# Purpurax/mcaat

Hardware: AMD Instinct MI355X
Metric: k-mers/sec through sdbg_build+cycle_finder, 1B-node graph @ 1/2/4/8 GPUs (higher is better)
Workload: dtype u64

## Files before the change

mcaat_amd/csrc/node_counter.hip:

```cpp
#include <hipcub/hipcub.hpp>

#include <algorithm>
#include <cstdio>
#include <cstdlib>
#include <ctime>
#include <functional>
#include <memory>
#include <mutex>
#include <type_traits>

#include "desc_canon.h"
#include "internal.h"

namespace mcaat {

namespace {

constexpr int kBlock = 256;


struct SkParams {
    int E;
    int m;
    int w;
    int nmax;
    int l2_bits;
    uint64_t salt;
    uint32_t mini;
};

__device__ __forceinline__ uint64_t desc_window(uint64_t w0, uint64_t w1, int i, int E) {
    uint64_t v;
    if (i == 0) v = w0;
    else if (i < 32) v = (w0 >> (2 * i)) | (w1 << (64 - 2 * i));
    else v = w1 >> (2 * (i - 32));
    return v & mask_bits(2 * E);
}

__device__ __forceinline__ uint32_t rev2_32(uint32_t x) {
    x = ((x >> 2) & 0x33333333u) | ((x & 0x33333333u) << 2);
    x = ((x >> 4) & 0x0F0F0F0Fu) | ((x & 0x0F0F0F0Fu) << 4);
    return __builtin_bswap32(x);
}
__device__ __forceinline__ uint32_t mix32(uint32_t x) {
    x ^= x >> 16;
    x *= 0x7feb352du;
    x ^= x >> 15;
    x *= 0x846ca68bu;
    x ^= x >> 16;
    return x;
}

__device__ __forceinline__ uint32_t part_mix(uint32_t h) { return mix32(h ^ 0x70617274u); }

__device__ __forceinline__ uint64_t canon_edge(uint64_t lsb, int E) {
    const uint64_t y = __builtin_bitreverse64(lsb);
    const uint64_t r2 = ((y >> 1) & 0x5555555555555555ULL) | ((y & 0x5555555555555555ULL) << 1);
    const uint64_t rc = (r2 >> (64 - 2 * E)) ^ mask_bits(2 * E);
    return lsb < rc ? lsb : rc;
}

#ifndef MCAAT_AWAVES
#define MCAAT_AWAVES 4
#define MCAAT_ASEG 900
#define MCAAT_APERCU 3
#endif
#ifndef MCAAT_HASH
#define MCAAT_HASH 2
#endif
constexpr int kAWaves = MCAAT_AWAVES;
constexpr int kAThreads = kAWaves * 64;
constexpr int kAPerCu = MCAAT_APERCU;
constexpr int kItem = 127;
constexpr int kCk = 8;
constexpr int kSeg = MCAAT_ASEG;
constexpr int kStage = kSeg * kAWaves;
static_assert(kAThreads >= 256, "threads < 256 own one L1 bucket each");
static_assert(kSeg > 64 * kCk, "a segment must hold a worst-case step");
static_assert(kStage <= 65536, "perm holds 16-bit stage indices");

struct ItemSrc {
    const uint64_t *offsets;
    uint64_t n_reads;
    uint64_t fixed_len;
    uint64_t ipr;
    const uint64_t *item_base;
    const uint32_t *item_np;
    uint64_t n_items;
};

__device__ __forceinline__ void get_item(const ItemSrc &s, int E, uint64_t it, uint64_t &base, int &np) {
    if (s.fixed_len) {
        const uint64_t r = it / s.ipr, c = it - r * s.ipr;
        const uint64_t npos = s.fixed_len - E + 1;
        base = r * s.fixed_len + c * kItem;
        const uint64_t rem = npos - c * kItem;
        np = (int)(rem < (uint64_t)kItem ? rem : kItem);
    } else {
        base = s.item_base[it];
        np = (int)s.item_np[it];
    }
}

struct __attribute__((aligned(8))) u64x2 {
    uint64_t a, b;
};

__device__ __forceinline__ uint64_t rev2_dev(uint64_t x) {
    const uint32_t lo = __builtin_bitreverse32((uint32_t)(x >> 32)), hi = __builtin_bitreverse32((uint32_t)x);
    const uint32_t l = ((lo >> 1) & 0x55555555u) | ((lo << 1) & 0xAAAAAAAAu);
    const uint32_t h = ((hi >> 1) & 0x55555555u) | ((hi << 1) & 0xAAAAAAAAu);
    return ((uint64_t)h << 32) | l;
}

__device__ __forceinline__ uint64_t win32(uint64_t a, uint64_t b, uint64_t B) {
    const int sh = 2 * (int)(B & 31);
    return sh ? (a >> sh) | (b << (64 - sh)) : a;
}

#ifndef MCAAT_HTOP
#define MCAAT_HTOP 1
#endif
template <bool FULL>
__device__ __forceinline__ void hash_step(uint64_t win, int m, uint32_t mmask, uint32_t salt, uint32_t *h) {
#if MCAAT_HTOP
    const int lo = 32 - 2 * m;
    const uint64_t Wt = win << lo;
    const uint64_t R = rev2_dev(win) ^ ~0ULL;
    const uint32_t wl = (uint32_t)Wt, wh = (uint32_t)(Wt >> 32);
    const uint32_t rl = (uint32_t)R, rh = (uint32_t)(R >> 32);
    (void)mmask;
#pragma unroll
    for (int t = 0; t < kCk; ++t) {
        const uint32_t f = t ? __builtin_amdgcn_alignbit(wh, wl, 2 * t) : wl;
        const uint32_t r = t ? __builtin_amdgcn_alignbit(rh, rl, 32 - 2 * t) : rh;
        const uint32_t c = FULL ? min(f, r) : min(f, r) >> lo;
#if MCAAT_HASH == 2
        h[t] = (c ^ salt) * 0x9E3779B1u;
#elif MCAAT_HASH == 1
        uint32_t x = (c ^ salt) * 0x9E3779B1u;
        h[t] = x ^ (x >> 15);
#else
        h[t] = mix32(c ^ salt);
#endif
    }
#else
    const uint64_t R = (rev2_dev(win) ^ ~0ULL) >> (2 * (25 - m));
    const uint32_t wl = (uint32_t)win, wh = (uint32_t)(win >> 32);
    const uint32_t rl = (uint32_t)R, rh = (uint32_t)(R >> 32);
#pragma unroll
    for (int t = 0; t < kCk; ++t) {
        uint32_t f = __builtin_amdgcn_alignbit(wh, wl, 2 * t);
        uint32_t r = __builtin_amdgcn_alignbit(rh, rl, 2 * (kCk - 1 - t));
        if (!FULL) {
            f &= mmask;
            r &= mmask;
        }
#if MCAAT_HASH == 2
        h[t] = (min(f, r) ^ salt) * 0x9E3779B1u;
#elif MCAAT_HASH == 1
        uint32_t x = (min(f, r) ^ salt) * 0x9E3779B1u;
        h[t] = x ^ (x >> 15);
#else
        h[t] = mix32(min(f, r) ^ salt);
#endif
    }
#endif
}

template <int W, int G>
__device__ __forceinline__ void window_min(const uint32_t *H, uint32_t *hm) {
    auto at = [&](int u) { return H[(G * kCk + u) % (3 * kCk)]; };
    if constexpr (W > kCk) {
        uint32_t S[kCk], Pm[W - 1];
        S[kCk - 1] = at(kCk - 1);
#pragma unroll
        for (int t = kCk - 2; t >= 0; --t) S[t] = min(at(t), S[t + 1]);
        Pm[0] = at(kCk);
#pragma unroll
        for (int u = 1; u < W - 1; ++u) Pm[u] = min(Pm[u - 1], at(kCk + u));
#pragma unroll
        for (int t = 0; t < kCk; ++t) hm[t] = min(S[t], Pm[t + W - 1 - kCk]);
    } else {
#pragma unroll
        for (int t = 0; t < kCk; ++t) {
            uint32_t v = at(t);
#pragma unroll
            for (int q = 1; q < W; ++q) v = min(v, at(t + q));
            hm[t] = v;
        }
    }
}

constexpr uint32_t kMiniOne = 1024, kMiniShard = 256;
constexpr uint16_t kDeadSub = 0xffff;


#ifndef MCAAT_WB
#define MCAAT_WB 4
#endif
#ifndef MCAAT_APF
#define MCAAT_APF 1
#endif
constexpr int kAPF = MCAAT_APF;
constexpr int kWB = MCAAT_WB;
#ifndef MCAAT_WPIPE
#define MCAAT_WPIPE 0
#endif
#ifndef MCAAT_CLOSEMASK
#define MCAAT_CLOSEMASK 1
#endif
constexpr bool kWPipe = MCAAT_WPIPE != 0;

constexpr int kPeP = 7, kPePar = 14, kPeLane = 15;

template <int W, bool FULL>
__global__ void __launch_bounds__(kAThreads) k_sk_scatter(const uint64_t *__restrict__ packed, ItemSrc src,
                                                          SkParams P, uint4 *__restrict__ l1_data,
                                                          const uint64_t *__restrict__ l1_base,
                                                          const uint64_t *__restrict__ l1_cap,
                                                          unsigned long long *l1_cursor, uint16_t *__restrict__ l1_sub,
                                                          unsigned long long *prof, unsigned long long *rstate, int rmode) {
    __shared__ uint64_t stage[kStage];
    __shared__ uint8_t stage_l1[kStage];
    __shared__ uint16_t perm[kStage];
    __shared__ uint64_t sbase[kAWaves][2][64];
    __shared__ uint32_t hist[256];
    __shared__ uint32_t boff[256];
    __shared__ uint32_t bcur[256];
    __shared__ unsigned long long rpos[256];
    __shared__ unsigned long long rlim[256];
    __shared__ uint32_t rleft[256];
    __shared__ uint32_t wtot[kAWaves];
    __shared__ int more_flag[2];

    const int wave = threadIdx.x >> 6, lane = threadIdx.x & 63;
    const int tb = threadIdx.x;
    unsigned long long my_next = 0, my_base = 0;
    uint32_t prev_need = 0;
    unsigned long long *rs = rstate ? rstate + ((uint64_t)blockIdx.x * 256 + (tb & 255)) * 3 : nullptr;
    if (tb < 256) {
        hist[tb] = 0;
        bcur[tb] = 0;
        my_base = l1_base[tb];
        rlim[tb] = my_base + l1_cap[tb];
        if (rmode >= 2) {
            rpos[tb] = rs[0];
            rleft[tb] = (uint32_t)rs[1];
            my_next = rs[2];
        } else {
            rleft[tb] = 0;
            my_next = atomicAdd(&l1_cursor[tb], (unsigned long long)P.mini);
        }
    }
    if (threadIdx.x == 0) more_flag[0] = more_flag[1] = 0;
    __syncthreads();
    uint64_t *seg = stage + __builtin_amdgcn_readfirstlane(wave * kSeg);
    uint8_t *seg_l1 = stage_l1 + wave * kSeg;
    uint32_t nflush = 0;

    const int sub_shift = kHShift + kHBits - P.l2_bits;
    auto put = [&](int b, uint64_t pos, const uint4 &d) {
        if (pos < rlim[b]) {
            l1_data[pos] = d;
            const uint64_t hi = (uint64_t)d.w << 32;
            l1_sub[pos] = ((d.w >> (kNShift - 32)) & 63) ? (uint16_t)(sub_shift < 64 ? hi >> sub_shift : 0) : kDeadSub;
        }
    };

    const uint64_t n_items = src.fixed_len ? src.n_reads * src.ipr : src.n_items;
    const uint64_t n_batches = (n_items + 63) / 64;
    const uint64_t bstride = (uint64_t)gridDim.x * kAWaves;
    uint64_t batch = (uint64_t)blockIdx.x * kAWaves + wave;
    constexpr bool kFull = FULL;
    const uint32_t mmask = (uint32_t)mask_bits(2 * P.m);
    const uint32_t salt32 = (uint32_t)P.salt;
    const int nmax = P.nmax;

    uint32_t H[3 * kCk];
    uint64_t cw[3], pa = 0, pb = 0;
    uint64_t qa = 0, qb = 0;
    uint64_t s = 0;
    int np = 0, c = 0, ph = 0, nck = 0;
    uint32_t prev_hm = 0, h_open = 0, p7 = 0, ihc = 0, fill = 0, par = 1, bsf = 0;
    bool active = false;
    auto fetch = [&](uint64_t bt, uint64_t &sb, int &n, uint64_t *w) {
        const uint64_t item = bt * 64 + lane;
        sb = 0;
        n = 0;
        if (bt < n_batches && item < n_items) get_item(src, P.E, item, sb, n);
#pragma unroll
        for (int k = 0; k < 3; ++k) w[k] = packed[(sb >> 5) + k];
    };

    auto step = [&](auto Gc) {
        constexpr int G = decltype(Gc)::value;
        c = __builtin_amdgcn_readfirstlane(c);
        const int rb = kCk * c + 2 * kCk;
        const uint64_t win = win32(pa, pb, s + rb);
        if constexpr (kAPF == 2) {
            pa = qa;
            pb = qb;
            const u64x2 nx = *(const u64x2 *)(packed + ((s + rb + 2 * kCk) >> 5));
            qa = nx.a;
            qb = nx.b;
        } else {
            const u64x2 nx = *(const u64x2 *)(packed + ((s + rb + kCk) >> 5));
            pa = nx.a;
            pb = nx.b;
        }
        hash_step<kFull>(win, P.m, mmask, salt32, H + ((G + 2) % 3) * kCk);
        uint32_t hm[kCk];
        window_min<W, G>(H, hm);
        if (c == 0) {
            prev_hm = hm[0];
            h_open = hm[0];
            p7 = 0;
        }
#if MCAAT_CLOSEMASK
        fill = __builtin_amdgcn_readfirstlane(fill);
#pragma unroll
        for (int t = 0; t < kCk; ++t) {
            const int i = kCk * c + t;
            const uint32_t prv = t ? hm[t - 1] : prev_hm;
            const unsigned long long bm = __builtin_amdgcn_ballot_w64((uint32_t)(i - 1) < (uint32_t)np) &
                                          (__builtin_amdgcn_ballot_w64(i == np) |
                                           __builtin_amdgcn_ballot_w64(hm[t] != prv) |
                                           __builtin_amdgcn_ballot_w64((int)p7 <= (i - nmax) * 128));
            if (bm) {
                if (__builtin_amdgcn_inverse_ballot_w64(bm)) {
                    const uint32_t idx =
                        __builtin_amdgcn_mbcnt_hi((uint32_t)(bm >> 32), __builtin_amdgcn_mbcnt_lo((uint32_t)bm, 0u));
                    seg[fill + idx] = ((uint64_t)(p7 + ihc + (uint32_t)i) << 32) | prv;
                    p7 = (uint32_t)i << kPeP;
                }
                fill += (uint32_t)__popcll(bm);
            }
        }
        (void)h_open;
#else
#pragma unroll
        for (int t = 0; t < kCk; ++t) {
            const int i = kCk * c + t;
            const uint32_t prv = t ? hm[t - 1] : prev_hm;
            const bool cl = ((uint32_t)(i - 1) < (uint32_t)np) &
                            ((i == np) | (hm[t] != prv) | ((int)p7 <= (i - nmax) * 128));
            const unsigned long long bm = __builtin_amdgcn_ballot_w64(cl);
            if (bm) {
                if (cl) {
                    const uint32_t idx =
                        __builtin_amdgcn_mbcnt_hi((uint32_t)(bm >> 32), __builtin_amdgcn_mbcnt_lo((uint32_t)bm, fill));
                    seg[idx] = ((uint64_t)(p7 + ihc + (uint32_t)i) << 32) | h_open;
                    p7 = (uint32_t)i << kPeP;
                    h_open = hm[t];
                }
                fill += (uint32_t)__popcll(bm);
            }
        }
#endif
        prev_hm = hm[kCk - 1];
    };

    unsigned long long tp[5] = {0, 0, 0, 0, 0}, t0 = prof ? __builtin_amdgcn_s_memrealtime() : 0;
    auto tick = [&](int phase) {
        if (prof) {
            const unsigned long long t1 = __builtin_amdgcn_s_memrealtime();
            tp[phase] += t1 - t0;
            t0 = t1;
        }
    };

    auto start_item = [&](auto Gc) {
        constexpr int G = decltype(Gc)::value;
        fetch(batch, s, np, cw);
        par ^= 1u;
        ++bsf;
        sbase[wave][par][lane] = s;
        ihc = (par << kPePar) | ((uint32_t)lane << kPeLane);
        {
            const u64x2 nx = *(const u64x2 *)(packed + ((s + 2 * kCk) >> 5));
            pa = nx.a;
            pb = nx.b;
        }
        if constexpr (kAPF == 2) {
            const u64x2 nx = *(const u64x2 *)(packed + ((s + 3 * kCk) >> 5));
            qa = nx.a;
            qb = nx.b;
        }
        int mx = np;
#pragma unroll
        for (int o = 32; o; o >>= 1) mx = max(mx, __shfl_xor(mx, o));
        nck = mx / kCk + 1;
        const int o8 = (int)(s & 31) + kCk;
        hash_step<kFull>(win32(cw[0], cw[1], s), P.m, mmask, salt32, H + G * kCk);
        hash_step<kFull>(o8 >= 32 ? win32(cw[1], cw[2], s + kCk) : win32(cw[0], cw[1], s + kCk), P.m, mmask,
                         salt32, H + ((G + 1) % 3) * kCk);
        c = 0;
        active = true;
    };
    auto run = [&](auto Gc) -> bool {
        constexpr int G = decltype(Gc)::value;
        if (!active) {
            if (batch >= n_batches || bsf >= 2) {
                ph = G;
                return false;
            }
            start_item(Gc);
        }
        if (fill + 64 * kCk > (uint32_t)kSeg) {
            ph = G;
            return false;
        }
        step(Gc);
        if (++c == nck) {
            active = false;
            batch += bstride;
        }
        return true;
    };

    for (;;) {
        ph = __builtin_amdgcn_readfirstlane(ph);
        if (ph != 0) {
            uint32_t T[3 * kCk];
#pragma unroll
            for (int u = 0; u < 3 * kCk; ++u) T[u] = H[u];
            if (ph == 1) {
#pragma unroll
                for (int u = 0; u < 3 * kCk; ++u) H[u] = T[(u + kCk) % (3 * kCk)];
            } else {
#pragma unroll
                for (int u = 0; u < 3 * kCk; ++u) H[u] = T[(u + 2 * kCk) % (3 * kCk)];
            }
            ph = 0;
        }
        for (;;) {
            if (!run(std::integral_constant<int, 0>())) break;
            if (!run(std::integral_constant<int, 1>())) break;
            if (!run(std::integral_constant<int, 2>())) break;
        }
        tick(0);
        for (uint32_t e = lane; e < fill; e += 64) {
            const uint32_t l1 = part_mix((uint32_t)seg[e]) >> 24;
            seg_l1[e] = (uint8_t)l1;
            atomicAdd(&hist[l1], 1u);
        }
        tick(1);
        if (lane == 0) wtot[wave] = fill;
        if (lane == 0 && (active || batch < n_batches)) more_flag[nflush & 1] = 1;
        lds_barrier();
        const int more = more_flag[nflush & 1];
        if (threadIdx.x == 0) more_flag[(nflush + 1) & 1] = 0;
        ++nflush;
        tick(2);
        if (tb < 256) {
            rpos[tb] += prev_need;
            rleft[tb] -= prev_need;
            const uint32_t need = hist[tb];
            if (need > rleft[tb]) {
                for (uint32_t z = 0; z < rleft[tb]; ++z) put(tb, rpos[tb] + z, make_uint4(0, 0, 0, 0));
                if (need <= P.mini) {
                    rpos[tb] = my_base + my_next;
                    rleft[tb] = P.mini;
                    my_next = atomicAdd(&l1_cursor[tb], (unsigned long long)P.mini);
                } else {
                    const uint32_t grab = ((need + P.mini - 1) / P.mini) * P.mini;
                    rpos[tb] = my_base + atomicAdd(&l1_cursor[tb], (unsigned long long)grab);
                    rleft[tb] = grab;
                }
            }
            prev_need = need;
        }
        if (wave == 0) {
            const uint4 hv = *(const uint4 *)&hist[4 * lane];
            const uint32_t sum4 = hv.x + hv.y + hv.z + hv.w;
            uint32_t incl = sum4;
#pragma unroll
            for (int o = 1; o < 64; o <<= 1) {
                const uint32_t v = __shfl_up(incl, o);
                if (lane >= o) incl += v;
            }
            const uint32_t ex = incl - sum4;
            *(uint4 *)&boff[4 * lane] = make_uint4(ex, ex + hv.x, ex + hv.x + hv.y, ex + hv.x + hv.y + hv.z);
        }
        lds_barrier();
        if (tb < 256) hist[tb] = 0;
        tick(3);
        for (uint32_t e = lane; e < fill; e += 64) {
            const int b = seg_l1[e];
            perm[boff[b] + atomicAdd(&bcur[b], 1u)] = (uint16_t)(wave * kSeg + e);
        }
        lds_barrier();
        uint32_t total = 0;
#pragma unroll
        for (int w = 0; w < kAWaves; ++w) total += wtot[w];
        uint64_t q[2][kWB], B0[2][kWB], x[2][kWB][3];
        auto load_batch = [&](auto Sc, uint32_t j0) {
            constexpr int S = decltype(Sc)::value;
#pragma unroll
            for (int k = 0; k < kWB; ++k) {
                const uint32_t j = j0 + k * kAThreads;
                q[S][k] = 0;
                B0[S][k] = 0;
                if (j < total) {
                    const uint32_t i = perm[j];
                    q[S][k] = stage[i];
                    const uint32_t hi = (uint32_t)(q[S][k] >> 32);
                    const uint32_t ln = (hi >> kPeLane) & 63, pr = (hi >> kPePar) & 1;
                    B0[S][k] = sbase[i / kSeg][pr][ln] + ((hi >> kPeP) & 127);
                }
                const int L = (int)(((uint32_t)(q[S][k] >> 32) & 127) - (((uint32_t)(q[S][k] >> 32) >> kPeP) & 127)) + P.E - 1;
                const u64x2 x01 = *(const u64x2 *)(packed + (B0[S][k] >> 5));
                x[S][k][0] = x01.a;
                x[S][k][1] = x01.b;
                x[S][k][2] = j < total && 2 * (int)(B0[S][k] & 31) + 2 * L > 128 ? packed[(B0[S][k] >> 5) + 2] : 0;
            }
        };
        auto store_batch = [&](auto Sc, uint32_t j0) {
            constexpr int S = decltype(Sc)::value;
#pragma unroll
            for (int k = 0; k < kWB; ++k) {
                const uint32_t j = j0 + k * kAThreads;
                if (j >= total) continue;
                const uint32_t i = perm[j];
                const int b = stage_l1[i];
                const uint32_t hi = (uint32_t)(q[S][k] >> 32);
                const uint32_t n = (hi & 127) - ((hi >> kPeP) & 127);
                const int sh = 2 * (int)(B0[S][k] & 31);
                const int L = (int)n + P.E - 1;
                const uint64_t w0 = (sh ? (x[S][k][0] >> sh) | (x[S][k][1] << (64 - sh)) : x[S][k][0]) & mask_bits(2 * L);
                uint64_t w1 = (sh ? (x[S][k][1] >> sh) | (x[S][k][2] << (64 - sh)) : x[S][k][1]) &
                              mask_bits(L > 32 ? 2 * (L - 32) : 0);
                const uint32_t h = part_mix((uint32_t)q[S][k]);
                w1 |= ((uint64_t)n << kNShift) | ((uint64_t)((h >> (24 - kHBits)) & ((1u << kHBits) - 1)) << kHShift);
                put(b, rpos[b] + (j - boff[b]),
                    make_uint4((uint32_t)w0, (uint32_t)(w0 >> 32), (uint32_t)w1, (uint32_t)(w1 >> 32)));
            }
        };
        constexpr uint32_t kStep = kWB * kAThreads;
        using S0 = std::integral_constant<int, 0>;
        using S1 = std::integral_constant<int, 1>;
        if constexpr (kWPipe) {
            uint32_t j0 = threadIdx.x;
            if (j0 < total) load_batch(S0(), j0);
            for (; j0 < total; j0 += 2 * kStep) {
                if (j0 + kStep < total) load_batch(S1(), j0 + kStep);
                store_batch(S0(), j0);
                if (j0 + kStep >= total) break;
                if (j0 + 2 * kStep < total) load_batch(S0(), j0 + 2 * kStep);
                store_batch(S1(), j0 + kStep);
            }
        } else {
            for (uint32_t j0 = threadIdx.x; j0 < total; j0 += kStep) {
                load_batch(S0(), j0);
                store_batch(S0(), j0);
            }
        }
        if (tb < 256) bcur[tb] = 0;
        fill = 0;
        bsf = active ? 1u : 0u;
        lds_barrier();
        tick(4);
        if (!more) break;
    }
    if (tb < 256) {
        rpos[tb] += prev_need;
        rleft[tb] -= prev_need;
    }
    if (rmode == 1 || rmode == 2) {
        if (tb < 256) {
            rs[0] = rpos[tb];
            rs[1] = rleft[tb];
            rs[2] = my_next;
        }
        return;
    }
    __syncthreads();
    for (int pass = 0; pass < 2; ++pass) {
        for (int b = 0; b < 256; ++b)
            for (uint32_t z = threadIdx.x; z < rleft[b]; z += kAThreads) put(b, rpos[b] + z, make_uint4(0, 0, 0, 0));
        __syncthreads();
        if (tb < 256) {
            rpos[tb] = my_base + my_next;
            rleft[tb] = P.mini;
        }
        __syncthreads();
    }
    if (prof && lane == 0)
        for (int i = 0; i < 5; ++i) atomicAdd(&prof[i], tp[i]);
}

typedef void (*SkKernel)(const uint64_t *, ItemSrc, SkParams, uint4 *, const uint64_t *, const uint64_t *,
                         unsigned long long *, uint16_t *, unsigned long long *, unsigned long long *, int);
SkKernel sk_kernel(int w, bool full) {
    if (full) {
        switch (w) {
#define MCAAT_SK(W) \
    case W:         \
        return k_sk_scatter<W, true>;
            MCAAT_SK(9) MCAAT_SK(10) MCAAT_SK(11) MCAAT_SK(12) MCAAT_SK(13) MCAAT_SK(14) MCAAT_SK(15) MCAAT_SK(16)
#undef MCAAT_SK
        }
    } else {
        switch (w) {
#define MCAAT_SK(W) \
    case W:         \
        return k_sk_scatter<W, false>;
            MCAAT_SK(1) MCAAT_SK(2) MCAAT_SK(3) MCAAT_SK(4) MCAAT_SK(5) MCAAT_SK(6) MCAAT_SK(7) MCAAT_SK(8)
            MCAAT_SK(9) MCAAT_SK(10) MCAAT_SK(11) MCAAT_SK(12) MCAAT_SK(13) MCAAT_SK(14) MCAAT_SK(15) MCAAT_SK(16)
#undef MCAAT_SK
        }
    }
    throw Error(MCAAT_E_INVALID, "node_counter: minimizer window out of range");
}

constexpr int kBThreads = 1024;
constexpr uint32_t kChunk = 65536;


#ifndef MCAAT_BLG
#define MCAAT_BLG 4
#endif
constexpr int kLG = MCAAT_BLG;
static_assert(kLG == 2 || kLG == 4, "32-B or 64-B lines");
__device__ __forceinline__ uint32_t round4(uint32_t x) { return (x + kLG - 1) & ~(uint32_t)(kLG - 1); }

__device__ __forceinline__ void chunk_hist(const uint16_t *__restrict__ sub, uint64_t s0, uint32_t n, uint32_t *lh) {
    const uint4 *v = (const uint4 *)(sub + s0);
    const uint32_t n8 = n / 8;
    for (uint32_t i0 = threadIdx.x; i0 < n8; i0 += 4 * kBThreads) {
        uint4 q[4];
#pragma unroll
        for (int k = 0; k < 4; ++k) q[k] = i0 + k * kBThreads < n8 ? v[i0 + k * kBThreads] : make_uint4(~0u, ~0u, ~0u, ~0u);
#pragma unroll
        for (int k = 0; k < 4; ++k) {
            const uint32_t w[4] = {q[k].x, q[k].y, q[k].z, q[k].w};
#pragma unroll
            for (int j = 0; j < 4; ++j) {
                if ((w[j] & 0xffff) != kDeadSub) atomicAdd(&lh[w[j] & 0xffff], 1u);
                if ((w[j] >> 16) != kDeadSub) atomicAdd(&lh[w[j] >> 16], 1u);
            }
        }
    }
    for (uint32_t i = 8 * n8 + threadIdx.x; i < n; i += kBThreads) {
        const uint32_t x = sub[s0 + i];
        if (x != kDeadSub) atomicAdd(&lh[x], 1u);
    }
}

__global__ void __launch_bounds__(kBThreads) k_l2_hist(const uint16_t *__restrict__ sub, const uint64_t *chunk_start,
                                                       const uint32_t *chunk_len, const uint32_t *chunk_bucket,
                                                       int l2_bits, unsigned long long *tot, uint32_t *cc) {
    extern __shared__ uint32_t lh[];
    const uint32_t S = 1u << l2_bits;
    const uint64_t c = blockIdx.x;
    for (uint32_t i = threadIdx.x; i < S; i += kBThreads) lh[i] = 0;
    __syncthreads();
    chunk_hist(sub, chunk_start[c], chunk_len[c], lh);
    __syncthreads();
    const uint64_t fb = (uint64_t)chunk_bucket[c] * S;
    for (uint32_t i = threadIdx.x; i < S; i += kBThreads) {
        cc[c * S + i] = lh[i];
        if (lh[i]) atomicAdd(&tot[fb + i], (unsigned long long)round4(lh[i]));
    }
}

__global__ void __launch_bounds__(256) k_chunk_runs(uint32_t *cc, const uint64_t *bchunk, const uint64_t *fine,
                                                    uint32_t S) {
    const uint64_t t = (uint64_t)blockIdx.x * blockDim.x + threadIdx.x;
    if (t >= 256ull * S) return;
    const uint64_t b = t / S, i = t % S;
    uint64_t run = fine[t] / kLG;
    for (uint64_t c = bchunk[b]; c < bchunk[b + 1]; ++c) {
        const uint32_t x = cc[c * S + i];
        cc[c * S + i] = (uint32_t)run;
        run += round4(x) / kLG;
    }
}

constexpr int kMaxSub = 2048;
#ifndef MCAAT_BPF
#define MCAAT_BPF 2
#endif
constexpr int kBPF = MCAAT_BPF;
#ifndef MCAAT_BCOOP
#define MCAAT_BCOOP 1
#endif
constexpr bool kCoopFlush = MCAAT_BCOOP != 0;

template <bool WEIGHTED>
__global__ void __launch_bounds__(kBThreads) k_l2_scatter(const uint4 *__restrict__ data,
                                                          const uint16_t *__restrict__ sub,
                                                          const uint64_t *chunk_start, const uint32_t *chunk_len,
                                                          const uint32_t *runs, int l2_bits, int E,
                                                          uint4 *__restrict__ out, uint64_t gbase,
                                                          const uint32_t *__restrict__ wgt,
                                                          uint32_t *__restrict__ out_w) {
    __shared__ uint4 buf[kMaxSub * kLG];
    __shared__ uint32_t lb[kMaxSub];
    __shared__ uint32_t lc[kMaxSub];
    __shared__ uint32_t bl[kMaxSub];
    const uint32_t S = 1u << l2_bits;
    const uint64_t c = blockIdx.x;
    for (uint32_t i = threadIdx.x; i < S; i += kBThreads) {
        lb[i] = runs[c * S + i];
        lc[i] = 0;
        bl[i] = 0;
    }
    __syncthreads();
    const uint64_t s0 = chunk_start[c];
    const uint32_t n = chunk_len[c];
    uint32_t v[kBPF];
    uint4 d[kBPF];
#pragma unroll
    for (int j = 0; j < kBPF; ++j) {
        const uint32_t i = j * kBThreads + threadIdx.x;
        v[j] = i < n ? sub[s0 + i] : kDeadSub;
        d[j] = i < n ? data[s0 + i] : make_uint4(0, 0, 0, 0);
    }
    for (uint32_t i00 = 0; i00 < n; i00 += kBPF * kBThreads)
#pragma unroll
    for (int j = 0; j < kBPF; ++j) {
        const uint32_t i0 = i00 + j * kBThreads;
        if (i0 >= n) break;
        const uint32_t cv = v[j];
        uint4 cd = d[j];
        const uint32_t ni = i0 + kBPF * kBThreads + threadIdx.x;
        v[j] = ni < n ? sub[s0 + ni] : kDeadSub;
        if (ni < n) d[j] = data[s0 + ni];
        const bool live = cv != kDeadSub;
        uint32_t r = 0, line = 0;
        bool buffered = false;
        if (live) {
            r = atomicAdd(&lc[cv], 1u);
            line = bl[cv];
            if constexpr (WEIGHTED) out_w[(uint64_t)lb[cv] * kLG + r - gbase] = wgt[s0 + i0 + threadIdx.x];
            uint64_t w0 = (uint64_t)cd.x | ((uint64_t)cd.y << 32), w1 = (uint64_t)cd.z | ((uint64_t)cd.w << 32);
            desc_canonical(w0, w1, E);
            cd = make_uint4((uint32_t)w0, (uint32_t)(w0 >> 32), (uint32_t)w1, (uint32_t)(w1 >> 32));
            buffered = r / kLG == line;
            if (buffered) buf[cv * kLG + (r & (kLG - 1))] = cd;
            else out[(uint64_t)lb[cv] * kLG + r - gbase] = cd;
        }
        lds_barrier();
        uint32_t nline = 0;
        if (kCoopFlush) {
            const bool done = live && buffered && (r & (kLG - 1)) == kLG - 1;
            const unsigned long long dm = __ballot(done);
            const uint32_t lane = threadIdx.x & 63;
            const uint64_t dst = done ? ((uint64_t)lb[cv] + line) * kLG - gbase : 0;
            const uint32_t src = done ? cv * kLG : 0;
            const int nd = __popcll(dm);
            for (int b0 = 0; b0 < nd; b0 += 64 / kLG) {
                const int j = b0 + (int)(lane / kLG);
                int pos = 0;
                if (j < nd) {
#pragma unroll
                    for (int step = 32; step; step >>= 1) {
                        const unsigned long long below = dm & ((pos + step >= 64) ? ~0ull : ((1ull << (pos + step)) - 1));
                        if (__popcll(below) <= j) pos += step;
                    }
                }
                const uint64_t d = __shfl(dst, pos);
                const uint32_t sidx = __shfl(src, pos);
                if (j < nd) out[d + (lane & (kLG - 1))] = buf[sidx + (lane & (kLG - 1))];
            }
            if (live) {
                nline = lc[cv] / kLG;
                bl[cv] = nline;
            }
        } else if (live) {
            if (buffered && (r & (kLG - 1)) == kLG - 1) {
                uint4 *o = out + (((uint64_t)lb[cv] + line) * kLG - gbase);
#pragma unroll
                for (int z = 0; z < kLG; ++z) o[z] = buf[cv * kLG + z];
            }
            nline = lc[cv] / kLG;
            bl[cv] = nline;
        }
        lds_barrier();
        if (live && !buffered && r / kLG == nline) buf[cv * kLG + (r & (kLG - 1))] = cd;
    }
    lds_barrier();
    for (uint32_t i = threadIdx.x; i < S; i += kBThreads) {
        const uint32_t k = lc[i];
        if (k & (kLG - 1)) {
            uint4 *o = out + (((uint64_t)lb[i] + k / kLG) * kLG - gbase);
#pragma unroll
            for (uint32_t z = 0; z < kLG; ++z) o[z] = z < (k & (kLG - 1)) ? buf[i * kLG + z] : make_uint4(0, 0, 0, 0);
            if constexpr (WEIGHTED)
                for (uint32_t z = k & (kLG - 1); z < kLG; ++z) out_w[((uint64_t)lb[i] + k / kLG) * kLG - gbase + z] = 0;
        }
    }
}

#ifndef MCAAT_CTHREADS
#define MCAAT_CTHREADS 1024
#endif
constexpr int kCThreads = MCAAT_CTHREADS;
constexpr int kCWaves = kCThreads / 64;
constexpr int kCap = 4096;
constexpr int kCapMax = kCap * 85 / 100 - kCWaves * 64;
constexpr int kDCap = 2048;
constexpr int kDMax = kDCap * 3 / 4;
constexpr int kDProbe = 128;
#ifndef MCAAT_CB
#define MCAAT_CB 1
#endif
constexpr int kCB = MCAAT_CB;
#ifndef MCAAT_CPF
#define MCAAT_CPF 1
#endif
constexpr bool kCPF = MCAAT_CPF != 0;
#ifndef MCAAT_CPERCU
#define MCAAT_CPERCU 2
#endif
constexpr int kCPerCu = MCAAT_CPERCU;
#ifndef MCAAT_CSPLIT
#define MCAAT_CSPLIT 2
#endif
constexpr uint32_t kSplitLg = MCAAT_CSPLIT;
static_assert(kSplitLg <= 3, "the sub-partition takes the top 11 of the 14 stored hash bits");
constexpr uint32_t kSplitMax = 3;
#ifndef MCAAT_CRING
#define MCAAT_CRING 0
#endif
constexpr int kCRing = MCAAT_CRING;
__device__ __forceinline__ void dma16(const uint4 *src, uint4 *lds) {
    const uint32_t dst = __builtin_amdgcn_readfirstlane(
        (uint32_t)(uintptr_t)(__attribute__((address_space(3))) void *)lds);
    uint32_t keep;
    asm volatile("s_mov_b32 %0, m0\n\ts_mov_b32 m0, %2\n\ts_nop 0\n\tglobal_load_lds_dwordx4 %1, off\n\ts_mov_b32 m0, %0"
                 : "=&s"(keep) : "v"(src), "s"(dst) : "memory");
}
__device__ __forceinline__ void wait_vm0() { asm volatile("s_waitcnt vmcnt(0)" ::: "memory"); }
__device__ __forceinline__ void wait_vm1() { asm volatile("s_waitcnt vmcnt(1)" ::: "memory"); }
// ... 1417 lines not shown
```

Measured before the change: 143.4 billion.

## Hold item bases in registers and store the partition hash in the stage entry

Each lane's item bases are now loaded once into ten 32-bit registers, and the per-step windows are built with alignbit and register shifts. This replaces the per-step global loads from the packed array. Item metadata and words are prefetched two batches ahead through an inline-asm register rotation. The stage_l1 byte array is dropped: part_mix is computed once and written back into the stage entry's low word, so the write phase no longer recomputes it, and the freed LDS allows a larger segment (1036). Uniform values are forced scalar with readfirstlane. The costs are higher register pressure and fragile inline asm.

```diff
diff --git a/mcaat_amd/csrc/node_counter.hip b/mcaat_amd/csrc/node_counter.hip
--- a/mcaat_amd/csrc/node_counter.hip
+++ b/mcaat_amd/csrc/node_counter.hip
@@ -60,9 +60,17 @@
     return lsb < rc ? lsb : rc;
 }
 
+#ifndef MCAAT_AREG
+#define MCAAT_AREG 1
+#endif
+#ifndef MCAAT_A1HASH
+#define MCAAT_A1HASH 1
+#endif
 #ifndef MCAAT_AWAVES
 #define MCAAT_AWAVES 4
-#define MCAAT_ASEG 900
+#ifndef MCAAT_ASEG
+#define MCAAT_ASEG (MCAAT_A1HASH ? 1036 : 900)
+#endif
 #define MCAAT_APERCU 3
 #endif
 #ifndef MCAAT_HASH
@@ -78,6 +86,12 @@
 static_assert(kAThreads >= 256, "threads < 256 own one L1 bucket each");
 static_assert(kSeg > 64 * kCk, "a segment must hold a worst-case step");
 static_assert(kStage <= 65536, "perm holds 16-bit stage indices");
+constexpr int kALds = kStage * (8 + 2 + (MCAAT_A1HASH ? 0 : 1)) + kAWaves * 2 * 64 * 8 + 3 * 256 * 4 +
+                      2 * 256 * 8 + 256 * 4 + kAWaves * 4 + 2 * 4;
+static_assert(kALds <= 160 * 1024 / kAPerCu, "kAPerCu workgroups of pass A must fit a CU's LDS");
+constexpr int kItemRegs = 10;
+static_assert(kItem + 32 - 1 <= 160, "an item's bases (E <= 32) fit five 64-bit words");
+static_assert(16 * kItemRegs == 160 && kCk == 8, "a step's window starts at a register or half way into one");
 
 struct ItemSrc {
     const uint64_t *offsets;
@@ -88,6 +102,18 @@
     const uint32_t *item_np;
     uint64_t n_items;
 };
+
+#if MCAAT_AREG
+__device__ __forceinline__ uint32_t uni(uint32_t x) { return __builtin_amdgcn_readfirstlane(x); }
+__device__ __forceinline__ int uni(int x) { return __builtin_amdgcn_readfirstlane(x); }
+__device__ __forceinline__ uint64_t uni64(uint64_t x) {
+    return ((uint64_t)uni((uint32_t)(x >> 32)) << 32) | uni((uint32_t)x);
+}
+#else
+__device__ __forceinline__ uint32_t uni(uint32_t x) { return x; }
+__device__ __forceinline__ int uni(int x) { return x; }
+__device__ __forceinline__ uint64_t uni64(uint64_t x) { return x; }
+#endif
 
 __device__ __forceinline__ void get_item(const ItemSrc &s, int E, uint64_t it, uint64_t &base, int &np) {
     if (s.fixed_len) {
@@ -202,7 +228,7 @@
 #ifndef MCAAT_APF
 #define MCAAT_APF 1
 #endif
-constexpr int kAPF = MCAAT_APF;
+[[maybe_unused]] constexpr int kAPF = MCAAT_APF;
 constexpr int kWB = MCAAT_WB;
 #ifndef MCAAT_WPIPE
 #define MCAAT_WPIPE 0
@@ -222,7 +248,9 @@
                                                           unsigned long long *l1_cursor, uint16_t *__restrict__ l1_sub,
                                                           unsigned long long *prof, unsigned long long *rstate, int rmode) {
     __shared__ uint64_t stage[kStage];
+#if !MCAAT_A1HASH
     __shared__ uint8_t stage_l1[kStage];
+#endif
     __shared__ uint16_t perm[kStage];
     __shared__ uint64_t sbase[kAWaves][2][64];
     __shared__ uint32_t hist[256];
@@ -256,7 +284,9 @@
     if (threadIdx.x == 0) more_flag[0] = more_flag[1] = 0;
     __syncthreads();
     uint64_t *seg = stage + __builtin_amdgcn_readfirstlane(wave * kSeg);
+#if !MCAAT_A1HASH
     uint8_t *seg_l1 = stage_l1 + wave * kSeg;
+#endif
     uint32_t nflush = 0;
 
     const int sub_shift = kHShift + kHBits - P.l2_bits;
@@ -278,12 +308,36 @@
     const int nmax = P.nmax;
 
     uint32_t H[3 * kCk];
+#if MCAAT_AREG
+    uint32_t iw[kItemRegs - 1];
+    u64x2 nraw[3] = {{0, 0}, {0, 0}, {0, 0}};
+    uint64_t s1 = 0, s2 = 0;
+    int np1 = 0, np2 = 0;
+#pragma unroll
+    for (int i = 0; i < kItemRegs - 1; ++i) iw[i] = 0;
+#else
     uint64_t cw[3], pa = 0, pb = 0;
     uint64_t qa = 0, qb = 0;
+#endif
     uint64_t s = 0;
     int np = 0, c = 0, ph = 0, nck = 0;
     uint32_t prev_hm = 0, h_open = 0, p7 = 0, ihc = 0, fill = 0, par = 1, bsf = 0;
     bool active = false;
+#if MCAAT_AREG
+    auto fetch_item = [&](uint64_t bt, uint64_t &sb, int &n) {
+        const uint64_t item = bt * 64 + lane;
+        sb = 0;
+        n = 0;
+        if (bt < n_batches && item < n_items) get_item(src, P.E, item, sb, n);
+    };
+    auto fetch_words = [&](uint64_t bt, uint64_t sb) {
+        if (bt < n_batches) {
+            const u64x2 *w = (const u64x2 *)(packed + (sb >> 5));
+#pragma unroll
+            for (int k = 0; k < 3; ++k) nraw[k] = w[k];
+        }
+    };
+#else
     auto fetch = [&](uint64_t bt, uint64_t &sb, int &n, uint64_t *w) {
         const uint64_t item = bt * 64 + lane;
         sb = 0;
@@ -292,10 +346,21 @@
 #pragma unroll
         for (int k = 0; k < 3; ++k) w[k] = packed[(sb >> 5) + k];
     };
+#endif
 
     auto step = [&](auto Gc) {
         constexpr int G = decltype(Gc)::value;
         c = __builtin_amdgcn_readfirstlane(c);
+#if MCAAT_AREG
+        const uint32_t wsh = (uint32_t)(c & 1) * 16;
+        const uint64_t win = ((uint64_t)__builtin_amdgcn_alignbit(iw[2], iw[1], wsh) << 32) |
+                             __builtin_amdgcn_alignbit(iw[1], iw[0], wsh);
+        if (c & 1) {
+#pragma unroll
+            for (int i = 0; i + 1 < kItemRegs - 1; ++i) iw[i] = iw[i + 1];
+            iw[kItemRegs - 2] = 0;
+        }
+#else
         const int rb = kCk * c + 2 * kCk;
         const uint64_t win = win32(pa, pb, s + rb);
         if constexpr (kAPF == 2) {
@@ -309,6 +374,7 @@
             pa = nx.a;
             pb = nx.b;
         }
+#endif
         hash_step<kFull>(win, P.m, mmask, salt32, H + ((G + 2) % 3) * kCk);
         uint32_t hm[kCk];
         window_min<W, G>(H, hm);
@@ -372,11 +438,53 @@
 
     auto start_item = [&](auto Gc) {
         constexpr int G = decltype(Gc)::value;
+#if MCAAT_AREG
+        s = s1;
+        np = np1;
+        uint32_t it0;
+        {
+            const uint32_t h[12] = {(uint32_t)nraw[0].a, (uint32_t)(nraw[0].a >> 32), (uint32_t)nraw[0].b,
+                                    (uint32_t)(nraw[0].b >> 32), (uint32_t)nraw[1].a, (uint32_t)(nraw[1].a >> 32),
+                                    (uint32_t)nraw[1].b, (uint32_t)(nraw[1].b >> 32), (uint32_t)nraw[2].a,
+                                    (uint32_t)(nraw[2].a >> 32), (uint32_t)nraw[2].b, (uint32_t)(nraw[2].b >> 32)};
+            const uint32_t lsh = 2 * ((uint32_t)s & 15);
+            const bool up = ((uint32_t)s & 16) != 0;
+            uint32_t t[kItemRegs + 1];
+#pragma unroll
+            for (int i = 0; i < kItemRegs + 1; ++i) t[i] = __builtin_amdgcn_alignbit(h[i + 1], h[i], lsh);
+            it0 = up ? t[1] : t[0];
+#pragma unroll
+            for (int i = 0; i < kItemRegs - 1; ++i) iw[i] = up ? t[i + 2] : t[i + 1];
+        }
+        static_assert(kItemRegs == 10, "the operand list below names every item register");
+        {
+            uint32_t lo, hi;
+            asm volatile("v_mov_b32 %0, %12\n\tv_mov_b32 %1, %13\n\tv_mov_b32 %2, %14"
+                         : "=&v"(lo), "=&v"(hi), "=&v"(np1), "+v"(it0), "+v"(iw[0]), "+v"(iw[1]), "+v"(iw[2]),
+                           "+v"(iw[3]), "+v"(iw[4]), "+v"(iw[5]), "+v"(iw[6]), "+v"(iw[7])
+                         : "v"((uint32_t)s2), "v"((uint32_t)(s2 >> 32)), "v"(np2), "v"(iw[8]));
+            s1 = ((uint64_t)hi << 32) | lo;
+        }
+        __builtin_amdgcn_sched_barrier(0);
+        fetch_words(batch + bstride, s1);
+        fetch_item(batch + 2 * bstride, s2, np2);
+#else
         fetch(batch, s, np, cw);
+#endif
         par ^= 1u;
         ++bsf;
         sbase[wave][par][lane] = s;
         ihc = (par << kPePar) | ((uint32_t)lane << kPeLane);
+        int mx = np;
+#pragma unroll
+        for (int o = 32; o; o >>= 1) mx = max(mx, __shfl_xor(mx, o));
+        nck = uni(mx / kCk + 1);
+#if MCAAT_AREG
+        hash_step<kFull>(((uint64_t)iw[0] << 32) | it0, P.m, mmask, salt32, H + G * kCk);
+        hash_step<kFull>(((uint64_t)__builtin_amdgcn_alignbit(iw[1], iw[0], 16) << 32) |
+                             __builtin_amdgcn_alignbit(iw[0], it0, 16),
+                         P.m, mmask, salt32, H + ((G + 1) % 3) * kCk);
+#else
         {
             const u64x2 nx = *(const u64x2 *)(packed + ((s + 2 * kCk) >> 5));
             pa = nx.a;
@@ -387,27 +495,25 @@
             qa = nx.a;
             qb = nx.b;
         }
-        int mx = np;
-#pragma unroll
-        for (int o = 32; o; o >>= 1) mx = max(mx, __shfl_xor(mx, o));
-        nck = mx / kCk + 1;
         const int o8 = (int)(s & 31) + kCk;
         hash_step<kFull>(win32(cw[0], cw[1], s), P.m, mmask, salt32, H + G * kCk);
         hash_step<kFull>(o8 >= 32 ? win32(cw[1], cw[2], s + kCk) : win32(cw[0], cw[1], s + kCk), P.m, mmask,
                          salt32, H + ((G + 1) % 3) * kCk);
+#endif
         c = 0;
         active = true;
     };
     auto run = [&](auto Gc) -> bool {
         constexpr int G = decltype(Gc)::value;
-        if (!active) {
-            if (batch >= n_batches || bsf >= 2) {
+        batch = uni64(batch);
+        if (!uni((int)active)) {
+            if (batch >= n_batches || uni(bsf) >= 2) {
                 ph = G;
                 return false;
             }
             start_item(Gc);
         }
-        if (fill + 64 * kCk > (uint32_t)kSeg) {
+        if (uni(fill) + 64 * kCk > (uint32_t)kSeg) {
             ph = G;
             return false;
         }
@@ -419,6 +525,11 @@
         return true;
     };
 
+#if MCAAT_AREG
+    fetch_item(batch, s1, np1);
+    fetch_words(batch, s1);
+    fetch_item(batch + bstride, s2, np2);
+#endif
     for (;;) {
         ph = __builtin_amdgcn_readfirstlane(ph);
         if (ph != 0) {
@@ -440,11 +551,20 @@
             if (!run(std::integral_constant<int, 2>())) break;
         }
         tick(0);
+#if MCAAT_A1HASH
+        for (uint32_t e = lane; e < fill; e += 64) {
+            uint32_t *lo = (uint32_t *)(seg + e);
+            const uint32_t pm = part_mix(*lo);
+            *lo = pm;
+            atomicAdd(&hist[pm >> 24], 1u);
+        }
+#else
         for (uint32_t e = lane; e < fill; e += 64) {
             const uint32_t l1 = part_mix((uint32_t)seg[e]) >> 24;
             seg_l1[e] = (uint8_t)l1;
             atomicAdd(&hist[l1], 1u);
         }
+#endif
         tick(1);
         if (lane == 0) wtot[wave] = fill;
         if (lane == 0 && (active || batch < n_batches)) more_flag[nflush & 1] = 1;
@@ -487,7 +607,11 @@
         if (tb < 256) hist[tb] = 0;
         tick(3);
         for (uint32_t e = lane; e < fill; e += 64) {
+#if MCAAT_A1HASH
+            const int b = (int)(*(const uint32_t *)(seg + e) >> 24);
+#else
             const int b = seg_l1[e];
+#endif
             perm[boff[b] + atomicAdd(&bcur[b], 1u)] = (uint16_t)(wave * kSeg + e);
         }
         lds_barrier();
@@ -522,8 +646,13 @@
             for (int k = 0; k < kWB; ++k) {
                 const uint32_t j = j0 + k * kAThreads;
                 if (j >= total) continue;
+#if MCAAT_A1HASH
+                const uint32_t h = (uint32_t)q[S][k];
+                const int b = (int)(h >> 24);
+#else
                 const uint32_t i = perm[j];
                 const int b = stage_l1[i];
+#endif
                 const uint32_t hi = (uint32_t)(q[S][k] >> 32);
                 const uint32_t n = (hi & 127) - ((hi >> kPeP) & 127);
                 const int sh = 2 * (int)(B0[S][k] & 31);
@@ -531,7 +660,9 @@
                 const uint64_t w0 = (sh ? (x[S][k][0] >> sh) | (x[S][k][1] << (64 - sh)) : x[S][k][0]) & mask_bits(2 * L);
                 uint64_t w1 = (sh ? (x[S][k][1] >> sh) | (x[S][k][2] << (64 - sh)) : x[S][k][1]) &
                               mask_bits(L > 32 ? 2 * (L - 32) : 0);
+#if !MCAAT_A1HASH
                 const uint32_t h = part_mix((uint32_t)q[S][k]);
+#endif
                 w1 |= ((uint64_t)n << kNShift) | ((uint64_t)((h >> (24 - kHBits)) & ((1u << kHBits) - 1)) << kHShift);
                 put(b, rpos[b] + (j - boff[b]),
                     make_uint4((uint32_t)w0, (uint32_t)(w0 >> 32), (uint32_t)w1, (uint32_t)(w1 >> 32)));
```

New measurement: 146.7 billion (median of 6 runs). +2.3%, better.
